# yycho0108/qpwcnet

Hardware: AMD Instinct MI355X
Metric: image-pairs/sec at 256x512 fp32 (higher is better)
Workload: dtype f32; 1 GPU; BASELINE configs[1]: full 6-level PWC-Net (qpwcnet build_flower) inference, batch 8 per GPU, 256x512 fp32, channels_last, d=4 cost volume + WarpV2; global_batch=8, batch_per_gpu=8, parallelism=dp1 (pairs sharded, RCCL all-gather of the 6 per-level EPE), hipgraph=True

## Files before the change

qpwcnet_amd/csrc/encoder.hip:

```cpp
#include "common.h"
#include "launch.h"

namespace qpwc {

__device__ __forceinline__ float enc_mishf(float x) {
    const float e = __builtin_amdgcn_exp2f(fminf(x, 20.0f) * 1.4426950408889634f);
    const float t = e * (e + 2.0f);
    const float m = x * (t * __builtin_amdgcn_rcpf(t + 2.0f));
    return m;
}

typedef float f32x4e __attribute__((ext_vector_type(4)));

__device__ __forceinline__ float2 ld2(const float* p) { return *reinterpret_cast<const float2*>(p); }
__device__ __forceinline__ float2 ld2(const __half* p) { return __half22float2(*reinterpret_cast<const __half2*>(p)); }
__device__ __forceinline__ void st4q(float* p, float4 v) { *reinterpret_cast<float4*>(p) = v; }
__device__ __forceinline__ void st4q(__half* p, float4 v) {
    __half2 lo = __floats2half2_rn(v.x, v.y), hi = __floats2half2_rn(v.z, v.w);
    uint2 u;
    u.x = *reinterpret_cast<unsigned*>(&lo);
    u.y = *reinterpret_cast<unsigned*>(&hi);
    *reinterpret_cast<uint2*>(p) = u;
}

constexpr int kEcTH = 8, kEcTW = 16;
constexpr int kEcHW = kEcTW + 2, kEcNH = (kEcTH + 2) * kEcHW;

template <int C>
__device__ __forceinline__ int ec_slot(int q, int hp) {
    return C == 16 ? (q ^ ((hp >> 2) & 3)) : (q ^ ((hp >> 1) & (C / 4 - 1)));
}

#ifndef QPWC_ENC_NT
#define QPWC_ENC_NT 1
#endif
#ifndef QPWC_UPCONV16_NFB_MIN_WGS
#define QPWC_UPCONV16_NFB_MIN_WGS 512
#endif
#ifndef QPWC_UPCONV256_TH
#define QPWC_UPCONV256_TH 2
#endif
#ifndef QPWC_UPCONV128_TH
#define QPWC_UPCONV128_TH 4
#endif
#ifndef QPWC_UPCONV64_LDS_TOTAL
#define QPWC_UPCONV64_LDS_TOTAL 82944
#endif
#ifndef QPWC_W_NEXT_ALWAYS
#define QPWC_W_NEXT_ALWAYS 1
#endif
#ifndef QPWC_W_NEXT_ALWAYS_F16
#define QPWC_W_NEXT_ALWAYS_F16 0
#endif
#if QPWC_W_NEXT_ALWAYS
#define QPWC_LOAD_W_NEXT(END) load_w(wn, kb + 1 < (END) ? kb + 1 : kb)
#else
#define QPWC_LOAD_W_NEXT(END) do { if (kb + 1 < (END)) load_w(wn, kb + 1); } while (0)
#endif
#ifdef QPWC_ENC_STAMP
__device__ long long g_enc_census[4096 * 6];
#define ENC_CENSUS(i) do { if (census_on) census_p[i] = __builtin_amdgcn_s_memtime(); } while (0)
#else
#define ENC_CENSUS(i) do { } while (0)
#endif
template <int C, int NT>
__global__ __launch_bounds__(256, 4) void conv3x3_mish_kernel(const float* __restrict__ x,
                                                              const float* __restrict__ weight,
                                                              const float* __restrict__ bias,
                                                              float* __restrict__ out, int H, int W,
                                                              int pad_h, int pad_w, int tiles_x, int tiles_y,
                                                              int groups_x) {
    constexpr int NQ = C / 4;
    constexpr int NFT = C / 16;
    constexpr int NKC = C / 16;
    constexpr int NLD = (kEcNH * NQ + 255) / 256;
    constexpr int NBUF = NT > 1 ? 2 : 1;
    __shared__ __attribute__((aligned(16))) float in_s[NBUF * kEcNH * C];
    const int tid0 = threadIdx.x;
    const int wave = __builtin_amdgcn_readfirstlane(tid0 >> 6);
    const int lane = tid0 & 63, n0 = lane & 15, g0 = lane >> 4;
    const int grp = xcd_swizzle(blockIdx.x, gridDim.x);
    const int gx0 = grp % groups_x, ty = (grp / groups_x) % tiles_y, b = grp / (groups_x * tiles_y);
    const int tx0 = gx0 * NT;
    const int Y0 = ty * kEcTH;
    const float* xb = x + (int64_t)b * H * W * C;
    const int Ho = H + pad_h, Wo = W + pad_w;
    float* ob = out + (int64_t)b * Ho * Wo * C;

    auto stage_load = [&](int tid, int tx, float4 (&v)[NLD]) {
        const int X0 = tx * kEcTW;
#pragma unroll
        for (int it = 0; it < NLD; ++it) {
            const int idx = tid + 256 * it;
            const int hp = idx / NQ, q = idx - hp * NQ;
            const int hy = hp / kEcHW, hx = hp - hy * kEcHW;
            const int gy = Y0 - 1 + hy, gx = X0 - 1 + hx;
            v[it] = (idx < kEcNH * NQ && gy >= 0 && gy < H && gx >= 0 && gx < W)
                        ? *reinterpret_cast<const float4*>(xb + ((int64_t)gy * W + gx) * C + 4 * q)
                        : make_float4(0.f, 0.f, 0.f, 0.f);
        }
    };
    auto stage_write = [&](int tid, int buf, const float4 (&v)[NLD]) {
#pragma unroll
        for (int it = 0; it < NLD; ++it) {
            const int idx = tid + 256 * it;
            const int hp = idx / NQ, q = idx - hp * NQ;
            if (idx < kEcNH * NQ)
                *reinterpret_cast<float4*>(in_s + buf * (kEcNH * C) + hp * C + 4 * ec_slot<C>(q, hp)) = v[it];
        }
    };
#ifdef QPWC_ENC_STAMP
    const bool census_on = tid0 == 0 && blockIdx.x < 4096;
    long long* census_p = g_enc_census + (blockIdx.x < 4096 ? blockIdx.x : 0) * 6;
    if (census_on)
        census_p[5] = (long long)(unsigned)__builtin_amdgcn_s_getreg((4) | (0 << 6) | (31 << 11)) |
                      ((long long)(unsigned)__builtin_amdgcn_s_getreg((20) | (0 << 6) | (31 << 11)) << 32);
#endif
    ENC_CENSUS(0);
    float4 st[NLD];
    stage_load(tid0, tx0, st);
#ifdef QPWC_ENC_STAMP
    asm volatile("s_waitcnt vmcnt(0)" ::: "memory");
#endif
    ENC_CENSUS(1);
    stage_write(tid0, 0, st);
    __syncthreads();
    ENC_CENSUS(2);

#pragma unroll 1
    for (int t = 0; t < NT; ++t) {
        const int tx = tx0 + t;
        if (tx >= tiles_x) break;
        const bool more = t + 1 < NT && tx + 1 < tiles_x;

        const int X0 = tx * kEcTW;
        const float* tile_s = in_s + (t & (NBUF - 1)) * (kEcNH * C);
        const float* wt = weight;
        int n = n0, g = g0, tid = tid0;
        if (NT > 1) asm volatile("" : "+r"(wt), "+v"(n), "+v"(g), "+v"(tid));
        if (more) stage_load(tid, tx + 1, st);
#pragma unroll
        for (int ft = 0; ft < NFT; ++ft) {
            f32x4e wld[9][NKC];
#pragma unroll
            for (int k = 0; k < 9; ++k)
#pragma unroll
                for (int kc = 0; kc < NKC; ++kc)
                    wld[k][kc] = *reinterpret_cast<const f32x4e*>(wt + ((int64_t)k * C + 16 * ft + n) * C + 16 * kc + 4 * g);
            f32x4e acc[2];
            acc[0] = f32x4e{0.f, 0.f, 0.f, 0.f};
            acc[1] = f32x4e{0.f, 0.f, 0.f, 0.f};
#pragma unroll
            for (int ky = 0; ky < 3; ++ky)
#pragma unroll
                for (int kx = 0; kx < 3; ++kx)
#pragma unroll
                    for (int kc = 0; kc < NKC; ++kc) {
                        f32x4e bv[2];
#pragma unroll
                        for (int m = 0; m < 2; ++m) {
                            const int hp = (2 * wave + m + ky) * kEcHW + n + kx;
                            const int q = 4 * kc + g;
                            const int slot = ec_slot<C>(q, hp);
                            bv[m] = *reinterpret_cast<const f32x4e*>(tile_s + hp * C + 4 * slot);
                        }
#pragma unroll
                        for (int tt = 0; tt < 4; ++tt)
#pragma unroll
                            for (int m = 0; m < 2; ++m)
                                acc[m] = __builtin_amdgcn_mfma_f32_16x16x4f32(wld[ky * 3 + kx][kc][tt], bv[m][tt], acc[m], 0, 0, 0);
                    }
            if (ft == NFT - 1) ENC_CENSUS(3);
            const float4 bq = *reinterpret_cast<const float4*>(bias + 16 * ft + 4 * g);
#pragma unroll
            for (int m = 0; m < 2; ++m) {
                const int gy = Y0 + 2 * wave + m, gx = X0 + n;
                if (gy < H && gx < W)
                    *reinterpret_cast<float4*>(ob + ((int64_t)gy * Wo + gx) * C + 16 * ft + 4 * g) =
                        make_float4(enc_mishf(acc[m][0] + bq.x), enc_mishf(acc[m][1] + bq.y),
                                    enc_mishf(acc[m][2] + bq.z), enc_mishf(acc[m][3] + bq.w));
            }
        }
        if (pad_w > 0 && X0 + kEcTW >= W) {
            for (int i = tid; i < kEcTH * pad_w * NQ; i += 256) {
                const int q = i % NQ, r = i / NQ, col = r % pad_w, row = r / pad_w;
                const int gy = Y0 + row;
                if (gy < H) *reinterpret_cast<float4*>(ob + ((int64_t)gy * Wo + W + col) * C + 4 * q) = make_float4(0.f, 0.f, 0.f, 0.f);
            }
        }
        if (pad_h > 0 && Y0 + kEcTH >= H) {
            const int x_end = (X0 + kEcTW >= W) ? Wo : X0 + kEcTW;
            for (int i = tid; i < pad_h * (x_end - X0) * NQ; i += 256) {
                const int q = i % NQ, r = i / NQ, col = r % (x_end - X0), row = r / (x_end - X0);
                *reinterpret_cast<float4*>(ob + ((int64_t)(H + row) * Wo + X0 + col) * C + 4 * q) = make_float4(0.f, 0.f, 0.f, 0.f);
            }
        }
        ENC_CENSUS(4);
        if (more) {
            stage_write(tid, (t + 1) & (NBUF - 1), st);
            __syncthreads();
        }
    }
}

constexpr int kEwSlots = 5;
constexpr unsigned kEwOob = 0x80000000u;

template <int C, int TH>
struct EwShape {
    static constexpr int NKB = C / 32;
    static constexpr int NS = 9 * NKB;
    static constexpr int NH = (TH + 2) * kEcHW;
    static constexpr int NHI = (NH * 8 + 255) / 256;
    static constexpr int HBLK = 4 * NHI * 1024;
    static constexpr int WBASE = 2 * HBLK;
    static constexpr int LDS = WBASE + 4 * kEwSlots * 2048;
    static_assert(NKB % 2 == 0, "the K-loop walks pairs of 32-channel blocks");
};

__device__ __forceinline__ void ew_wait_vm(int n) {
    switch (n) {
#define EW_W(k) case k: asm volatile("s_waitcnt vmcnt(" #k ")" ::: "memory"); break;
        EW_W(1) EW_W(2) EW_W(3) EW_W(4) EW_W(5) EW_W(6) EW_W(7) EW_W(8) EW_W(9) EW_W(10) EW_W(11) EW_W(12)
#undef EW_W
        default: asm volatile("s_waitcnt vmcnt(0)" ::: "memory"); break;
    }
}

__device__ __forceinline__ void ew_dma16(__amdgpu_buffer_rsrc_t r, char* lds, unsigned voff, int soff) {
#ifdef __HIP_DEVICE_COMPILE__
    typedef __attribute__((address_space(3))) void* lds_ptr_t;
    __builtin_amdgcn_raw_ptr_buffer_load_lds(r, (lds_ptr_t)lds, 16, voff, soff, 0, 0);
#endif
}

__device__ __forceinline__ void ew_pin_agpr(f32x4e& v) {
#ifdef __HIP_DEVICE_COMPILE__
    asm volatile("" : "+a"(v));
#endif
}

template <int C, int TH>
__global__ __launch_bounds__(256, (2 * EwShape<C, TH>::LDS <= 160 * 1024) ? 2 : 1) void conv3x3_mish_ring_kernel(
    const float* __restrict__ x, const float* __restrict__ weight, const float* __restrict__ bias,
    float* __restrict__ out, int H, int W, int pad_h, int pad_w, int tiles_x, int tiles_y, int n_tiles) {
    using S = EwShape<C, TH>;
    __shared__ __attribute__((aligned(1024))) char smem[S::LDS];
    const int tid = threadIdx.x;
    const int wave = __builtin_amdgcn_readfirstlane(tid >> 6);
    const int lane = tid & 63, n = lane & 15, g = lane >> 4;
    const int slice = blockIdx.x / n_tiles;
    const int tile = xcd_swizzle(blockIdx.x % n_tiles, n_tiles);
    const int tx = tile % tiles_x, ty = (tile / tiles_x) % tiles_y, b = tile / (tiles_x * tiles_y);
    const int X0 = tx * kEcTW, Y0 = ty * TH;
    const int fo = 64 * slice + 16 * wave;
    const __amdgpu_buffer_rsrc_t rx = __builtin_amdgcn_make_buffer_rsrc(
        const_cast<float*>(x) + (int64_t)b * H * W * C, 0, H * W * C * 4, 0x00020000);
    const __amdgpu_buffer_rsrc_t rw = __builtin_amdgcn_make_buffer_rsrc(const_cast<float*>(weight), 0, 9 * C * C * 4, 0x00020000);

    unsigned hoff[S::NHI];
#pragma unroll
    for (int j = 0; j < S::NHI; ++j) {
        const int i = (wave * S::NHI + j) * 64 + lane;
        const int hp = i >> 3, q = (i & 7) ^ (hp & 7);
        const int hy = hp / kEcHW, hx = hp - hy * kEcHW;
        const int gy = Y0 - 1 + hy, gx = X0 - 1 + hx;
        hoff[j] = (hp < S::NH && gy >= 0 && gy < H && gx >= 0 && gx < W) ? (unsigned)(((gy * W + gx) * C + 4 * q) * 4) : kEwOob;
    }
    const unsigned woff = (unsigned)(((fo + n) * C + 4 * g) * 4);
    auto issue_h = [&](int kb) __attribute__((always_inline)) {
#pragma unroll
        for (int j = 0; j < S::NHI; ++j)
            ew_dma16(rx, smem + (kb & 1) * S::HBLK + (wave * S::NHI + j) * 1024, hoff[j], kb * 128);
    };
    auto issue_w = [&](int s) __attribute__((always_inline)) {
        const int sc = s < S::NS ? s : S::NS - 1;
        const int kb = sc / 9, tap = sc - 9 * kb;
        char* dst = smem + S::WBASE + ((s % kEwSlots) * 4 + wave) * 2048;
#pragma unroll
        for (int kc = 0; kc < 2; ++kc)
            ew_dma16(rw, dst + kc * 1024, woff, (tap * C * C + 32 * kb + 16 * kc) * 4);
    };
    f32x4e wa[2][2], pb[2][2][TH];
    auto read = [&](int s, int buf) __attribute__((always_inline)) {
        const int kb = s / 9, tap = s - 9 * kb, ky = tap / 3, kx = tap - 3 * ky;
        const char* ws = smem + S::WBASE + ((s % kEwSlots) * 4 + wave) * 2048 + lane * 16;
        const char* hs = smem + (kb & 1) * S::HBLK;
#pragma unroll
        for (int kc = 0; kc < 2; ++kc) {
            wa[buf][kc] = *reinterpret_cast<const f32x4e*>(ws + kc * 1024);
#pragma unroll
            for (int m = 0; m < TH; ++m) {
                const int hp = (m + ky) * kEcHW + n + kx;
                pb[buf][kc][m] = *reinterpret_cast<const f32x4e*>(hs + hp * 128 + 16 * ((4 * kc + g) ^ (hp & 7)));
            }
        }
    };
    f32x4e acc[TH];
#pragma unroll
    for (int m = 0; m < TH; ++m) {
        acc[m] = f32x4e{0.f, 0.f, 0.f, 0.f};
        ew_pin_agpr(acc[m]);
    }

    issue_h(0);
#pragma unroll
    for (int s = 0; s < kEwSlots - 1; ++s) issue_w(s);
    ew_wait_vm(2 * (kEwSlots - 2));
    __builtin_amdgcn_s_barrier();
    read(0, 0);

    auto pair = [&](int p, const bool LAST) __attribute__((always_inline)) {
#pragma unroll
        for (int t = 0; t < 18; ++t) {
            const int s = 18 * p + t;
            const bool more = !(LAST && t == 17);
            if (more) {
                const int tb = t % 9;
                const bool h_young = tb >= 1 && tb <= kEwSlots - 2 && !(LAST && t >= 9);
                ew_wait_vm(2 * (kEwSlots - 3) + (h_young ? S::NHI : 0));
                if (tb == 8) {
                    asm volatile("s_waitcnt lgkmcnt(0)" ::: "memory");
                    __builtin_amdgcn_s_barrier();
                }
            }
            issue_w(s + kEwSlots - 1);
            if (t == 0) issue_h(2 * p + 1);
            if (t == 9 && !LAST) issue_h(2 * p + 2);
            if (more) read(s + 1, (t + 1) & 1);
            __builtin_amdgcn_sched_barrier(0);
#pragma unroll
            for (int kc = 0; kc < 2; ++kc)
#pragma unroll
                for (int tt = 0; tt < 4; ++tt)
#pragma unroll
                    for (int m = 0; m < TH; ++m)
                        acc[m] = __builtin_amdgcn_mfma_f32_16x16x4f32(wa[t & 1][kc][tt], pb[t & 1][kc][m][tt], acc[m], 0, 0, 0);
#pragma unroll
            for (int m = 0; m < TH; ++m) ew_pin_agpr(acc[m]);
            __builtin_amdgcn_sched_barrier(0);
        }
    };
#pragma unroll 1
    for (int p = 0; p < S::NKB / 2 - 1; ++p) pair(p, false);
    pair(S::NKB / 2 - 1, true);
    asm volatile("s_waitcnt vmcnt(0)" ::: "memory");

    const int Ho = H + pad_h, Wo = W + pad_w;
    float* ob = out + (int64_t)b * Ho * Wo * C;
    const float4 bq = *reinterpret_cast<const float4*>(bias + fo + 4 * g);
#pragma unroll
    for (int m = 0; m < TH; ++m) {
        const int gy = Y0 + m, gx = X0 + n;
        if (gy < H && gx < W)
            *reinterpret_cast<float4*>(ob + ((int64_t)gy * Wo + gx) * C + fo + 4 * g) =
                make_float4(enc_mishf(acc[m][0] + bq.x), enc_mishf(acc[m][1] + bq.y),
                            enc_mishf(acc[m][2] + bq.z), enc_mishf(acc[m][3] + bq.w));
    }
    if (pad_w > 0 && X0 + kEcTW >= W) {
        for (int i = tid; i < TH * pad_w * 16; i += 256) {
            const int q = i & 15, r = i >> 4, col = r % pad_w, row = r / pad_w;
            const int gy = Y0 + row;
            if (gy < H) *reinterpret_cast<float4*>(ob + ((int64_t)gy * Wo + W + col) * C + 64 * slice + 4 * q) = make_float4(0.f, 0.f, 0.f, 0.f);
        }
    }
    if (pad_h > 0 && Y0 + TH >= H) {
        const int x_end = (X0 + kEcTW >= W) ? Wo : X0 + kEcTW;
        for (int i = tid; i < pad_h * (x_end - X0) * 16; i += 256) {
            const int q = i & 15, r = i >> 4, col = r % (x_end - X0), row = r / (x_end - X0);
            *reinterpret_cast<float4*>(ob + ((int64_t)(H + row) * Wo + X0 + col) * C + 64 * slice + 4 * q) = make_float4(0.f, 0.f, 0.f, 0.f);
        }
    }
}

template <int C, int TH>
static int conv3x3_mish_ring_launch(const void* x, const void* weight, const void* bias, void* out, int B, int H,
                                    int W, int pad_h, int pad_w, hipStream_t s) {
    const int tiles_x = (W + kEcTW - 1) / kEcTW, tiles_y = (H + TH - 1) / TH;
    const int64_t n_tiles = (int64_t)tiles_x * tiles_y * B;
    if (n_tiles * (C / 64) > INT32_MAX || (int64_t)H * W * C * 4 > INT32_MAX) {
        set_error("conv3x3_mish: too many tiles or a frame of 2 GiB or more");
        return QPWC_E_SHAPE;
    }
    hipLaunchKernelGGL((conv3x3_mish_ring_kernel<C, TH>), dim3((unsigned)(n_tiles * (C / 64))), dim3(256), 0, s,
                       (const float*)x, (const float*)weight, (const float*)bias, (float*)out, H, W, pad_h, pad_w,
                       tiles_x, tiles_y, (int)n_tiles);
    return check_launch("conv3x3_mish_ring_kernel");
}

typedef _Float16 f16x8e __attribute__((ext_vector_type(8)));
typedef _Float16 f16x4e __attribute__((ext_vector_type(4)));

template <int CP>
__device__ __forceinline__ int f16_slot(int q, int hp) {
    return CP == 32 ? (q ^ ((0 - (hp >> 2)) & 3)) : (CP == 64 ? (q ^ ((hp >> 1) & 7)) : (q ^ (hp & 15)));
}

template <int C, int TH>
__global__ __launch_bounds__(256) void conv3x3_mish_f16_kernel(const __half* __restrict__ x,
                                                              const __half* __restrict__ weight,
                                                              const float* __restrict__ bias,
                                                              __half* __restrict__ out, int H, int W, int pad_h,
                                                              int pad_w, int tiles_x, int tiles_y, int n_tiles) {
    constexpr int CP = C < 32 ? 32 : C;
    constexpr int NQ = CP / 8, NQG = C / 8;
    constexpr int HH = TH + 2, NH = HH * kEcHW;
    constexpr int NKB = CP / 32;
    constexpr int FW = C < 64 ? C : 64, NFT = FW / 16, NSL = C / FW;
    constexpr int RW = TH / 4;
    constexpr int NST = (NH * NQ + 255) / 256;
    __shared__ __attribute__((aligned(16))) __half in_s[NH * CP];
    const int tid = threadIdx.x;
    const int wave = __builtin_amdgcn_readfirstlane(tid >> 6);
    const int lane = tid & 63, n = lane & 15, g = lane >> 4;
    const int slice = blockIdx.x / n_tiles;
    const int tile = xcd_swizzle(blockIdx.x % n_tiles, n_tiles);
    const int tx = tile % tiles_x, ty = (tile / tiles_x) % tiles_y, b = tile / (tiles_x * tiles_y);
    const int X0 = tx * kEcTW, Y0 = ty * TH;
    const int f0 = FW * slice;
    const __half* xb = x + (int64_t)b * H * W * C;
    {
        uint4 st[NST];
#pragma unroll
        for (int it = 0; it < NST; ++it) {
            const int idx = tid + 256 * it;
            const int hp = idx / NQ, q = idx - hp * NQ;
            const int hy = hp / kEcHW, hx = hp - hy * kEcHW;
            const int gy = Y0 - 1 + hy, gx = X0 - 1 + hx;
            st[it] = (idx < NH * NQ && q < NQG && gy >= 0 && gy < H && gx >= 0 && gx < W)
                         ? *reinterpret_cast<const uint4*>(xb + ((int64_t)gy * W + gx) * C + 8 * q)
                         : make_uint4(0u, 0u, 0u, 0u);
        }
#pragma unroll
        for (int it = 0; it < NST; ++it) {
            const int idx = tid + 256 * it;
            const int hp = idx / NQ, q = idx - hp * NQ;
            if (idx < NH * NQ) *reinterpret_cast<uint4*>(in_s + hp * CP + 8 * f16_slot<CP>(q, hp)) = st[it];
        }
    }
    const int Ho = H + pad_h, Wo = W + pad_w;
    __half* ob = out + (int64_t)b * Ho * Wo * C;
    if (C >= 64) {
        const int fo = f0 + 16 * wave;
        f32x4e acw[TH];
#pragma unroll
        for (int r = 0; r < TH; ++r) acw[r] = f32x4e{0.f, 0.f, 0.f, 0.f};
        f16x8e wv[9], wn[9];
        auto load_w = [&](f16x8e (&w)[9], int kb) {
#pragma unroll
            for (int tap = 0; tap < 9; ++tap)
                w[tap] = *reinterpret_cast<const f16x8e*>(weight + ((int64_t)tap * C + fo + n) * C + 32 * kb + 8 * g);
        };
        load_w(wv, 0);
        __syncthreads();
        auto block = [&](f16x8e (&wv)[9], int kb) __attribute__((always_inline)) {
            f16x8e bb[2][TH];
            auto read_b = [&](f16x8e (&bv)[TH], int tap) __attribute__((always_inline)) {
                const int ky = tap / 3, kx = tap - 3 * ky;
#pragma unroll
                for (int r = 0; r < TH; ++r) {
                    const int hp = (r + ky) * kEcHW + n + kx;
                    bv[r] = *reinterpret_cast<const f16x8e*>(in_s + hp * CP + 8 * f16_slot<CP>(4 * kb + g, hp));
                }
            };
            read_b(bb[0], 0);
#pragma unroll
            for (int tap = 0; tap < 9; ++tap) {
                if (tap + 1 < 9) read_b(bb[(tap + 1) & 1], tap + 1);
#pragma unroll
                for (int r = 0; r < TH; ++r)
                    acw[r] = __builtin_amdgcn_mfma_f32_16x16x32_f16(wv[tap], bb[tap & 1][r], acw[r], 0, 0, 0);
                __builtin_amdgcn_sched_barrier(0);
            }
        };
#if QPWC_W_NEXT_ALWAYS_F16
        {
            int kb = 0;
#pragma unroll 1
            for (; kb + 1 < NKB; kb += 2) {
                load_w(wn, kb + 1);
                __builtin_amdgcn_sched_barrier(0);
                block(wv, kb);
                load_w(wv, kb + 2 < NKB ? kb + 2 : kb);
                __builtin_amdgcn_sched_barrier(0);
                block(wn, kb + 1);
            }
            if (kb < NKB) block(wv, kb);
        }
#else
#pragma unroll 1
        for (int kb = 0; kb < NKB; ++kb) {
            if (kb + 1 < NKB) load_w(wn, kb + 1);
            block(wv, kb);
#pragma unroll
            for (int tap = 0; tap < 9; ++tap) wv[tap] = wn[tap];
        }
#endif
        const float4 bq = *reinterpret_cast<const float4*>(bias + fo + 4 * g);
#pragma unroll
        for (int r = 0; r < TH; ++r) {
            const int gy = Y0 + r, gx = X0 + n;
            if (gy < H && gx < W) {
                f16x4e o;
                o[0] = (_Float16)enc_mishf(acw[r][0] + bq.x);
                o[1] = (_Float16)enc_mishf(acw[r][1] + bq.y);
                o[2] = (_Float16)enc_mishf(acw[r][2] + bq.z);
                o[3] = (_Float16)enc_mishf(acw[r][3] + bq.w);
                *reinterpret_cast<f16x4e*>(ob + ((int64_t)gy * Wo + gx) * C + fo + 4 * g) = o;
            }
        }
    } else {
    f32x4e acc[RW][NFT];
#pragma unroll
    for (int r = 0; r < RW; ++r)
#pragma unroll
        for (int ft = 0; ft < NFT; ++ft) acc[r][ft] = f32x4e{0.f, 0.f, 0.f, 0.f};
    __syncthreads();
    const bool kvalid = 8 * g < C;
#pragma unroll 1
    for (int kb = 0; kb < NKB; ++kb) {
#pragma unroll
        for (int tap = 0; tap < 9; ++tap) {
            const int ky = tap / 3, kx = tap - 3 * ky;
            f16x8e wv[NFT];
#pragma unroll
            for (int ft = 0; ft < NFT; ++ft) {
                wv[ft] = f16x8e{0, 0, 0, 0, 0, 0, 0, 0};
                if (kvalid)
                    wv[ft] = *reinterpret_cast<const f16x8e*>(weight + ((int64_t)tap * C + f0 + 16 * ft + n) * C + 32 * kb + 8 * g);
            }
            f16x8e bv[RW];
#pragma unroll
            for (int r = 0; r < RW; ++r) {
                const int hp = (RW * wave + r + ky) * kEcHW + n + kx;
                bv[r] = *reinterpret_cast<const f16x8e*>(in_s + hp * CP + 8 * f16_slot<CP>(4 * kb + g, hp));
            }
#pragma unroll
            for (int ft = 0; ft < NFT; ++ft)
#pragma unroll
                for (int r = 0; r < RW; ++r)
                    acc[r][ft] = __builtin_amdgcn_mfma_f32_16x16x32_f16(wv[ft], bv[r], acc[r][ft], 0, 0, 0);
        }
    }
    float4 bqs[NFT];
#pragma unroll
    for (int ft = 0; ft < NFT; ++ft) bqs[ft] = *reinterpret_cast<const float4*>(bias + f0 + 16 * ft + 4 * g);
#pragma unroll
    for (int ft = 0; ft < NFT; ++ft) {
        const float4 bq = bqs[ft];
#pragma unroll
        for (int r = 0; r < RW; ++r) {
            const int gy = Y0 + RW * wave + r, gx = X0 + n;
            if (gy < H && gx < W) {
                f16x4e o;
                o[0] = (_Float16)enc_mishf(acc[r][ft][0] + bq.x);
                o[1] = (_Float16)enc_mishf(acc[r][ft][1] + bq.y);
                o[2] = (_Float16)enc_mishf(acc[r][ft][2] + bq.z);
                o[3] = (_Float16)enc_mishf(acc[r][ft][3] + bq.w);
                *reinterpret_cast<f16x4e*>(ob + ((int64_t)gy * Wo + gx) * C + f0 + 16 * ft + 4 * g) = o;
            }
        }
    }
    }
    constexpr int NQF = FW / 8;
    if (pad_w > 0 && X0 + kEcTW >= W) {
        for (int i = tid; i < TH * pad_w * NQF; i += 256) {
            const int q = i % NQF, r = i / NQF, col = r % pad_w, row = r / pad_w;
            const int gy = Y0 + row;
            if (gy < H) *reinterpret_cast<uint4*>(ob + ((int64_t)gy * Wo + W + col) * C + f0 + 8 * q) = make_uint4(0u, 0u, 0u, 0u);
        }
    }
    if (pad_h > 0 && Y0 + TH >= H) {
        const int x_end = (X0 + kEcTW >= W) ? Wo : X0 + kEcTW;
        for (int i = tid; i < pad_h * (x_end - X0) * NQF; i += 256) {
            const int q = i % NQF, r = i / NQF, col = r % (x_end - X0), row = r / (x_end - X0);
            *reinterpret_cast<uint4*>(ob + ((int64_t)(H + row) * Wo + X0 + col) * C + f0 + 8 * q) = make_uint4(0u, 0u, 0u, 0u);
        }
    }
    (void)NSL;
}

template <int C>
__device__ __forceinline__ int f16n_slot(int q, int hp) {
    return C == 16 ? (q ^ ((hp >> 3) & 1)) : (q ^ ((0 - (hp >> 2)) & 3));
}

template <int C>
__global__ __launch_bounds__(256, C == 16 ? 4 : 3) void conv3x3_mish_f16_narrow_kernel(
    const __half* __restrict__ x, const __half* __restrict__ weight, const float* __restrict__ bias,
    __half* __restrict__ out, int H, int W, int pad_h, int pad_w, int tiles_x, int tiles_y) {
    constexpr int TH = 16, RW = 4, HWD = kEcTW + 2;
    constexpr int NQ = C / 8, NH = (TH + 2) * HWD;
    constexpr int NST = (NH * NQ + 255) / 256;
    constexpr int NFT = C / 16;
    __shared__ __attribute__((aligned(16))) __half in_s[NH * C];
    const int tid = threadIdx.x;
    const int wave = __builtin_amdgcn_readfirstlane(tid >> 6);
    const int lane = tid & 63, n = lane & 15, g = lane >> 4;
    const int tile = xcd_swizzle(blockIdx.x, gridDim.x);
    const int tx = tile % tiles_x, ty = (tile / tiles_x) % tiles_y, b = tile / (tiles_x * tiles_y);
    const int X0 = tx * kEcTW, Y0 = ty * TH;
    const __half* xb = x + (int64_t)b * H * W * C;
    const int Ho = H + pad_h, Wo = W + pad_w;
    __half* ob = out + (int64_t)b * Ho * Wo * C;
    {
        uint4 st[NST];
#pragma unroll
        for (int it = 0; it < NST; ++it) {
            const int idx = tid + 256 * it;
            const int hp = idx / NQ, q = idx - hp * NQ;
            const int hy = hp / HWD, hx = hp - hy * HWD;
            const int gy = Y0 - 1 + hy, gx = X0 - 1 + hx;
            st[it] = (idx < NH * NQ && gy >= 0 && gy < H && gx >= 0 && gx < W)
                         ? *reinterpret_cast<const uint4*>(xb + ((int64_t)gy * W + gx) * C + 8 * q)
                         : make_uint4(0u, 0u, 0u, 0u);
        }
#pragma unroll
        for (int it = 0; it < NST; ++it) {
            const int idx = tid + 256 * it;
            const int hp = idx / NQ, q = idx - hp * NQ;
            if (idx < NH * NQ) *reinterpret_cast<uint4*>(in_s + hp * C + 8 * f16n_slot<C>(q, hp)) = st[it];
        }
    }
    constexpr int NS = C == 16 ? 5 : 9;
    const int gh = C == 16 ? (g >> 1) : 0, gq = C == 16 ? (g & 1) : g;
    f16x8e wv[NS][NFT];
#pragma unroll
    for (int j = 0; j < NS; ++j) {
        const int tap = C == 16 ? 2 * j + gh : j;
#pragma unroll
        for (int ft = 0; ft < NFT; ++ft) {
            wv[j][ft] = f16x8e{0, 0, 0, 0, 0, 0, 0, 0};
            if (tap < 9) wv[j][ft] = *reinterpret_cast<const f16x8e*>(weight + ((int64_t)tap * C + 16 * ft + n) * C + 8 * gq);
        }
    }
    f32x4e acc[RW][NFT];
#pragma unroll
    for (int r = 0; r < RW; ++r)
#pragma unroll
        for (int ft = 0; ft < NFT; ++ft) acc[r][ft] = f32x4e{0.f, 0.f, 0.f, 0.f};
    __syncthreads();
    f16x8e bb[2][RW];
    auto read_b = [&](f16x8e (&bv)[RW], int j) __attribute__((always_inline)) {
        const int t0 = C == 16 ? 2 * j + gh : j;
        const int tap = t0 < 9 ? t0 : 8;
        const int ky = tap / 3, kx = tap - 3 * ky;
#pragma unroll
        for (int r = 0; r < RW; ++r) {
            const int hp = (RW * wave + r + ky) * HWD + n + kx;
            bv[r] = *reinterpret_cast<const f16x8e*>(in_s + hp * C + 8 * f16n_slot<C>(gq, hp));
        }
    };
    read_b(bb[0], 0);
#pragma unroll
    for (int j = 0; j < NS; ++j) {
        if (j + 1 < NS) read_b(bb[(j + 1) & 1], j + 1);
#pragma unroll
        for (int ft = 0; ft < NFT; ++ft)
#pragma unroll
            for (int r = 0; r < RW; ++r)
                acc[r][ft] = __builtin_amdgcn_mfma_f32_16x16x32_f16(wv[j][ft], bb[j & 1][r], acc[r][ft], 0, 0, 0);
        __builtin_amdgcn_sched_barrier(0);
    }
    float4 bqs[NFT];
#pragma unroll
    for (int ft = 0; ft < NFT; ++ft) bqs[ft] = *reinterpret_cast<const float4*>(bias + 16 * ft + 4 * g);
#pragma unroll
    for (int ft = 0; ft < NFT; ++ft) {
        const float4 bq = bqs[ft];
#pragma unroll
        for (int r = 0; r < RW; ++r) {
            const int gy = Y0 + RW * wave + r, gx = X0 + n;
            if (gy < H && gx < W) {
                f16x4e o;
                o[0] = (_Float16)enc_mishf(acc[r][ft][0] + bq.x);
                o[1] = (_Float16)enc_mishf(acc[r][ft][1] + bq.y);
                o[2] = (_Float16)enc_mishf(acc[r][ft][2] + bq.z);
                o[3] = (_Float16)enc_mishf(acc[r][ft][3] + bq.w);
                *reinterpret_cast<f16x4e*>(ob + ((int64_t)gy * Wo + gx) * C + 16 * ft + 4 * g) = o;
            }
        }
    }
    if (pad_w > 0 && X0 + kEcTW >= W) {
        for (int i = tid; i < TH * pad_w * NQ; i += 256) {
            const int q = i % NQ, r = i / NQ, col = r % pad_w, row = r / pad_w;
            const int gy = Y0 + row;
            if (gy < H) *reinterpret_cast<uint4*>(ob + ((int64_t)gy * Wo + W + col) * C + 8 * q) = make_uint4(0u, 0u, 0u, 0u);
        }
    }
    if (pad_h > 0 && Y0 + TH >= H) {
// ... 543 lines not shown
            if (gy < Ho && gx < Wo)
                *reinterpret_cast<float4*>(ob + ((int64_t)gy * Wo + gx) * CO + 16 * ft + 4 * g) =
                    make_float4(enc_mishf(acc[m][ft][0] + bq.x), enc_mishf(acc[m][ft][1] + bq.y),
                                enc_mishf(acc[m][ft][2] + bq.z), enc_mishf(acc[m][ft][3] + bq.w));
        }
    }
}

template <int CI, int TH>
__global__ __launch_bounds__(256, (2 * (2 * TH + 1) * (kEcTW + 1) * CI * 4 > 80 * 1024) ? 1 : 2) void conv3x3s2_mish_wide_kernel(const float* __restrict__ x,
                                                                     const float* __restrict__ weight,
                                                                     const float* __restrict__ bias,
                                                                     float* __restrict__ out, int H, int W,
                                                                     int tiles_x, int tiles_y, int n_tiles) {
    constexpr int CO = 2 * CI, NQ = CI / 4, NKB = CI / 32;
    constexpr int IH = 2 * TH + 1, PW = kEcTW + 1;
    constexpr int NPX = IH * 33;
    constexpr int NST = (NPX * NQ + 255) / 256;
    __shared__ __attribute__((aligned(16))) float in_s[2 * IH * PW * CI];
    const int tid = threadIdx.x;
    const int wave = __builtin_amdgcn_readfirstlane(tid >> 6);
    const int lane = tid & 63, n = lane & 15, g = lane >> 4;
    const int slice = blockIdx.x / n_tiles;
    const int tile = xcd_swizzle(blockIdx.x % n_tiles, n_tiles);
    const int tx = tile % tiles_x, ty = (tile / tiles_x) % tiles_y, b = tile / (tiles_x * tiles_y);
    const int X0 = tx * kEcTW, Y0 = ty * TH;
    const int Hp = H + 1, Wp = W + 1, Ho = H / 2, Wo = W / 2;
    const int fo = 64 * slice + 16 * wave;
    const float* xb = x + (int64_t)b * Hp * Wp * CI;
    auto slot = [](int q, int pix) { return CI == 32 ? (q ^ ((pix >> 1) & 7)) : (q ^ (pix & 15)); };
    constexpr int kChunk = NST;
#pragma unroll
    for (int base = 0; base < NST; base += kChunk) {
        float4 st[kChunk];
#pragma unroll
        for (int i = 0; i < kChunk; ++i) {
            const int idx = tid + 256 * (base + i);
            const int pxl = idx / NQ, q = idx - pxl * NQ;
            const int row = pxl / 33, col = pxl - row * 33;
            const int gy = 2 * Y0 + row, gx = 2 * X0 + col;
            st[i] = (base + i < NST && idx < NPX * NQ && gy < Hp && gx < Wp)
                        ? *reinterpret_cast<const float4*>(xb + ((int64_t)gy * Wp + gx) * CI + 4 * q)
                        : make_float4(0.f, 0.f, 0.f, 0.f);
        }
#pragma unroll
        for (int i = 0; i < kChunk; ++i) {
            const int idx = tid + 256 * (base + i);
            const int pxl = idx / NQ, q = idx - pxl * NQ;
            const int row = pxl / 33, col = pxl - row * 33;
            const int pix = ((col & 1) * IH + row) * PW + (col >> 1);
            if (base + i < NST && idx < NPX * NQ) *reinterpret_cast<float4*>(in_s + pix * CI + 4 * slot(q, pix)) = st[i];
        }
    }
    f32x4e acc[TH];
#pragma unroll
    for (int m = 0; m < TH; ++m) acc[m] = f32x4e{0.f, 0.f, 0.f, 0.f};
    f32x4e wv[9][2], wn[9][2];
    auto load_w = [&](f32x4e (&w)[9][2], int kb) {
#pragma unroll
        for (int k = 0; k < 9; ++k)
#pragma unroll
            for (int kc = 0; kc < 2; ++kc)
                w[k][kc] = *reinterpret_cast<const f32x4e*>(weight + ((int64_t)k * CO + fo + n) * CI + 32 * kb + 16 * kc + 4 * g);
    };
    load_w(wv, 0);
    __syncthreads();
    auto block = [&](f32x4e (&wv)[9][2], int kb) __attribute__((always_inline)) {
#pragma unroll
        for (int ky = 0; ky < 3; ++ky)
#pragma unroll
            for (int kx = 0; kx < 3; ++kx)
#pragma unroll
                for (int kc = 0; kc < 2; ++kc) {
                    f32x4e bv[TH];
#pragma unroll
                    for (int m = 0; m < TH; ++m) {
                        const int pix = ((kx & 1) * IH + 2 * m + ky) * PW + n + (kx >> 1);
                        bv[m] = *reinterpret_cast<const f32x4e*>(in_s + pix * CI + 4 * slot(8 * kb + 4 * kc + g, pix));
                    }
#pragma unroll
                    for (int t = 0; t < 4; ++t)
#pragma unroll
                        for (int m = 0; m < TH; ++m)
                            acc[m] = __builtin_amdgcn_mfma_f32_16x16x4f32(wv[ky * 3 + kx][kc][t], bv[m][t], acc[m], 0, 0, 0);
                }
    };
#if QPWC_W_NEXT_ALWAYS
    {
        int kb = 0;
#pragma unroll 1
        for (; kb + 1 < NKB; kb += 2) {
            load_w(wn, kb + 1);
            __builtin_amdgcn_sched_barrier(0);
            block(wv, kb);
            load_w(wv, kb + 2 < NKB ? kb + 2 : kb);
            __builtin_amdgcn_sched_barrier(0);
            block(wn, kb + 1);
        }
        if (kb < NKB) block(wv, kb);
    }
#else
#pragma unroll 1
    for (int kb = 0; kb < NKB; ++kb) {
        if (kb + 1 < NKB) load_w(wn, kb + 1);
        block(wv, kb);
#pragma unroll
        for (int k = 0; k < 9; ++k)
#pragma unroll
            for (int kc = 0; kc < 2; ++kc) wv[k][kc] = wn[k][kc];
    }
#endif
    float* ob = out + (int64_t)b * Ho * Wo * CO;
    const float4 bq = *reinterpret_cast<const float4*>(bias + fo + 4 * g);
#pragma unroll
    for (int m = 0; m < TH; ++m) {
        const int gy = Y0 + m, gx = X0 + n;
        if (gy < Ho && gx < Wo)
            *reinterpret_cast<float4*>(ob + ((int64_t)gy * Wo + gx) * CO + fo + 4 * g) =
                make_float4(enc_mishf(acc[m][0] + bq.x), enc_mishf(acc[m][1] + bq.y),
                            enc_mishf(acc[m][2] + bq.z), enc_mishf(acc[m][3] + bq.w));
    }
}

template <int CI, int TH>
static int conv3x3s2_mish_wide_launch(const void* x, const void* weight, const void* bias, void* out, int B,
                                      int H, int W, hipStream_t s) {
    const int tiles_x = (W / 2 + kEcTW - 1) / kEcTW, tiles_y = (H / 2 + TH - 1) / TH;
    const int64_t n_tiles = (int64_t)tiles_x * tiles_y * B;
    const int slices = 2 * CI / 64;
    if (n_tiles * slices > INT32_MAX) {
        set_error("conv3x3s2_mish: too many tiles");
        return QPWC_E_SHAPE;
    }
    hipLaunchKernelGGL((conv3x3s2_mish_wide_kernel<CI, TH>), dim3((unsigned)(n_tiles * slices)), dim3(256), 0, s,
                       (const float*)x, (const float*)weight, (const float*)bias, (float*)out, H, W, tiles_x, tiles_y,
                       (int)n_tiles);
    return check_launch("conv3x3s2_mish_wide_kernel");
}

int conv3x3s2_mish_any_launch(const void* x, const void* weight, const void* bias, void* out, int B, int H, int W,
                              int CI, hipStream_t s);

int conv3x3s2_mish_launch(const void* x, const void* weight, const void* bias, void* out, int B, int H, int W,
                          hipStream_t s) {
    const int tiles_x = (W / 2 + kEcTW - 1) / kEcTW, tiles_y = (H / 2 + kEcTH - 1) / kEcTH;
    const int64_t nblk = (int64_t)tiles_x * tiles_y * B;
    if (nblk > INT32_MAX) {
        set_error("conv3x3s2_mish: too many tiles");
        return QPWC_E_SHAPE;
    }
    hipLaunchKernelGGL(conv3x3s2_mish_kernel, dim3((unsigned)nblk), dim3(256), 0, s, (const float*)x,
                       (const float*)weight, (const float*)bias, (float*)out, H, W, tiles_x, tiles_y);
    return check_launch("conv3x3s2_mish_kernel");
}

int conv3x3s2_mish_any_launch(const void* x, const void* weight, const void* bias, void* out, int B, int H, int W,
                              int CI, hipStream_t s) {
    switch (CI) {
        case 16: return conv3x3s2_mish_launch(x, weight, bias, out, B, H, W, s);
        case 32: return conv3x3s2_mish_wide_launch<32, 4>(x, weight, bias, out, B, H, W, s);
        case 64: return conv3x3s2_mish_wide_launch<64, 2>(x, weight, bias, out, B, H, W, s);
        case 128: return conv3x3s2_mish_wide_launch<128, 2>(x, weight, bias, out, B, H, W, s);
        default: set_error("conv3x3s2_mish: C_in=%d not in {16,32,64,128}", CI); return QPWC_E_SHAPE;
    }
}

template <int CI, int TH>
__global__ __launch_bounds__(256) void conv3x3s2_mish_f16_kernel(const __half* __restrict__ x,
                                                                const __half* __restrict__ weight,
                                                                const float* __restrict__ bias,
                                                                __half* __restrict__ out, int H, int W, int tiles_x,
                                                                int tiles_y, int n_tiles) {
    constexpr int CO = 2 * CI;
    constexpr int CP = CI < 32 ? 32 : CI;
    constexpr int NQ = CP / 8, NQG = CI / 8, NKB = CP / 32;
    constexpr int IH = 2 * TH + 1, PW = kEcTW + 1;
    constexpr int NB = CO / 16;
    constexpr int WB = NB < 4 ? NB : 4, WR = 4 / WB;
    constexpr int RW = TH / WR;
    constexpr int NCH = IH * (2 * kEcTW + 1) * NQ;
    constexpr int NST = (NCH + 255) / 256;
    __shared__ __attribute__((aligned(16))) __half in_s[2 * IH * PW * CP];
    const int tid = threadIdx.x;
    const int wave = __builtin_amdgcn_readfirstlane(tid >> 6);
    const int lane = tid & 63, n = lane & 15, g = lane >> 4;
    const int slice = blockIdx.x / n_tiles;
    const int tile = xcd_swizzle(blockIdx.x % n_tiles, n_tiles);
    const int tx = tile % tiles_x, ty = (tile / tiles_x) % tiles_y, b = tile / (tiles_x * tiles_y);
    const int X0 = tx * kEcTW, Y0 = ty * TH;
    const int Hp = H + 1, Wp = W + 1, Ho = H / 2, Wo = W / 2;
    const __half* xb = x + (int64_t)b * Hp * Wp * CI;
    {
        uint4 st[NST];
#pragma unroll
        for (int it = 0; it < NST; ++it) {
            const int idx = tid + 256 * it;
            const int q = idx % NQ, pc = idx / NQ;
            const int row = pc / (2 * kEcTW + 1), col = pc - row * (2 * kEcTW + 1);
            const int gy = 2 * Y0 + row, gx = 2 * X0 + col;
            st[it] = (idx < NCH && q < NQG && gy < Hp && gx < Wp)
                         ? *reinterpret_cast<const uint4*>(xb + ((int64_t)gy * Wp + gx) * CI + 8 * q)
                         : make_uint4(0u, 0u, 0u, 0u);
        }
#pragma unroll
        for (int it = 0; it < NST; ++it) {
            const int idx = tid + 256 * it;
            const int q = idx % NQ, pc = idx / NQ;
            const int row = pc / (2 * kEcTW + 1), col = pc - row * (2 * kEcTW + 1);
            const int hp = ((col & 1) * IH + row) * PW + (col >> 1);
            if (idx < NCH) *reinterpret_cast<uint4*>(in_s + hp * CP + 8 * f16_slot<CP>(q, hp)) = st[it];
        }
    }
    const int blk = WB == 4 ? 4 * slice + wave : (wave % WB);
    const int r0 = WB == 4 ? 0 : (wave / WB) * RW;
    const int fo = 16 * blk;
    f32x4e acc[RW];
#pragma unroll
    for (int r = 0; r < RW; ++r) acc[r] = f32x4e{0.f, 0.f, 0.f, 0.f};
    const bool kvalid = 8 * g < CI;
    f16x8e wv[9], wn[9];
    auto load_w = [&](f16x8e (&w)[9], int kb) {
#pragma unroll
        for (int tap = 0; tap < 9; ++tap) {
            w[tap] = f16x8e{0, 0, 0, 0, 0, 0, 0, 0};
            if (kvalid) w[tap] = *reinterpret_cast<const f16x8e*>(weight + ((int64_t)tap * CO + fo + n) * CI + 32 * kb + 8 * g);
        }
    };
    load_w(wv, 0);
    __syncthreads();
    auto block = [&](f16x8e (&wv)[9], int kb) __attribute__((always_inline)) {
#pragma unroll
        for (int tap = 0; tap < 9; ++tap) {
            const int ky = tap / 3, kx = tap - 3 * ky;
#pragma unroll
            for (int r = 0; r < RW; ++r) {
                const int hp = ((kx & 1) * IH + 2 * (r0 + r) + ky) * PW + n + (kx >> 1);
                const f16x8e bv = *reinterpret_cast<const f16x8e*>(in_s + hp * CP + 8 * f16_slot<CP>(4 * kb + g, hp));
                acc[r] = __builtin_amdgcn_mfma_f32_16x16x32_f16(wv[tap], bv, acc[r], 0, 0, 0);
            }
        }
    };
#if QPWC_W_NEXT_ALWAYS_F16
    {
        int kb = 0;
#pragma unroll 1
        for (; kb + 1 < NKB; kb += 2) {
            load_w(wn, kb + 1);
            __builtin_amdgcn_sched_barrier(0);
            block(wv, kb);
            load_w(wv, kb + 2 < NKB ? kb + 2 : kb);
            __builtin_amdgcn_sched_barrier(0);
            block(wn, kb + 1);
        }
        if (kb < NKB) block(wv, kb);
    }
#else
#pragma unroll 1
    for (int kb = 0; kb < NKB; ++kb) {
        if (kb + 1 < NKB) load_w(wn, kb + 1);
        block(wv, kb);
#pragma unroll
        for (int tap = 0; tap < 9; ++tap) wv[tap] = wn[tap];
    }
#endif
    __half* ob = out + (int64_t)b * Ho * Wo * CO;
    const float4 bq = *reinterpret_cast<const float4*>(bias + fo + 4 * g);
#pragma unroll
    for (int r = 0; r < RW; ++r) {
        const int gy = Y0 + r0 + r, gx = X0 + n;
        if (gy < Ho && gx < Wo)
            st4q(ob + ((int64_t)gy * Wo + gx) * CO + fo + 4 * g,
                 make_float4(enc_mishf(acc[r][0] + bq.x), enc_mishf(acc[r][1] + bq.y), enc_mishf(acc[r][2] + bq.z),
                             enc_mishf(acc[r][3] + bq.w)));
    }
}

template <int CI, int TH>
static int conv3x3s2_mish_f16_launch_t(const void* x, const void* weight, const void* bias, void* out, int B, int H,
                                       int W, hipStream_t s) {
    constexpr int NSL = (2 * CI / 16) < 4 ? 1 : (2 * CI / 16) / 4;
    const int tiles_x = (W / 2 + kEcTW - 1) / kEcTW, tiles_y = (H / 2 + TH - 1) / TH;
    const int64_t n_tiles = (int64_t)tiles_x * tiles_y * B;
    if (n_tiles * NSL > INT32_MAX) {
        set_error("conv3x3s2_mish_f16: too many tiles");
        return QPWC_E_SHAPE;
    }
    hipLaunchKernelGGL((conv3x3s2_mish_f16_kernel<CI, TH>), dim3((unsigned)(n_tiles * NSL)), dim3(256), 0, s,
                       (const __half*)x, (const __half*)weight, (const float*)bias, (__half*)out, H, W, tiles_x,
                       tiles_y, (int)n_tiles);
    return check_launch("conv3x3s2_mish_f16_kernel");
}

int conv3x3s2_mish_f16_launch(const void* x, const void* weight, const void* bias, void* out, int B, int H, int W,
                              int CI, hipStream_t s) {
    switch (CI) {
        case 16: return conv3x3s2_mish_f16_launch_t<16, 8>(x, weight, bias, out, B, H, W, s);
        case 32: return conv3x3s2_mish_f16_launch_t<32, 8>(x, weight, bias, out, B, H, W, s);
        case 64: return conv3x3s2_mish_f16_launch_t<64, 4>(x, weight, bias, out, B, H, W, s);
        case 128: return conv3x3s2_mish_f16_launch_t<128, 2>(x, weight, bias, out, B, H, W, s);
        default: set_error("conv3x3s2_mish_f16: C_in=%d not in {16,32,64,128}", CI); return QPWC_E_SHAPE;
    }
}

int conv3x3_mish_launch(const void* x, const void* weight, const void* bias, void* out, int B, int H, int W,
                        int C, int pad_h, int pad_w, hipStream_t s) {
    const int tiles_x = (W + kEcTW - 1) / kEcTW, tiles_y = (H + kEcTH - 1) / kEcTH;
    constexpr int NT = QPWC_ENC_NT;
    const int groups_x = (tiles_x + NT - 1) / NT;
    const int64_t nblk = (int64_t)groups_x * tiles_y * B;
    if (nblk > INT32_MAX) {
        set_error("conv3x3_mish: too many tiles");
        return QPWC_E_SHAPE;
    }
    const dim3 grid((unsigned)nblk);
    if (C == 16)
        hipLaunchKernelGGL((conv3x3_mish_kernel<16, NT>), grid, dim3(256), 0, s, (const float*)x, (const float*)weight,
                           (const float*)bias, (float*)out, H, W, pad_h, pad_w, tiles_x, tiles_y, groups_x);
    else if (C == 32)
        hipLaunchKernelGGL((conv3x3_mish_kernel<32, NT>), grid, dim3(256), 0, s, (const float*)x, (const float*)weight,
                           (const float*)bias, (float*)out, H, W, pad_h, pad_w, tiles_x, tiles_y, groups_x);
    else if (C == 64)
        return conv3x3_mish_ring_launch<64, 4>(x, weight, bias, out, B, H, W, pad_h, pad_w, s);
    else if (C == 128)
        return conv3x3_mish_ring_launch<128, 4>(x, weight, bias, out, B, H, W, pad_h, pad_w, s);
    else if (C == 256)
        return conv3x3_mish_ring_launch<256, 2>(x, weight, bias, out, B, H, W, pad_h, pad_w, s);
    else {
        set_error("conv3x3_mish: C=%d not in {16,32,64,128,256}", C);
        return QPWC_E_SHAPE;
    }
    return check_launch("conv3x3_mish_kernel");
}

}

#ifdef QPWC_ENC_STAMP
extern "C" int qpwc_debug_enc_census(long long* out, int n) {
    if (n > 4096 * 6) n = 4096 * 6;
    return (int)hipMemcpyFromSymbol(out, HIP_SYMBOL(qpwc::g_enc_census), n * sizeof(long long), 0, hipMemcpyDeviceToHost);
}
#endif
```

Baseline: 7327 pairs/s.

## Add persistent double-buffered MFMA conv3x3 Mish kernel for 16/32 channels

Adds a persistent-grid kernel for the C=16 and C=32 fp32 3x3 conv+Mish layers. Each workgroup loops over tiles and prefetches the next tile's halo into a second LDS slot via buffer DMA while computing the current one. Weights stay in registers and f32 MFMA 16x16x4 runs with swizzled LDS reads. The grid is capped at CUs times a fixed per-CU workgroup count. The aim is to hide global-load latency and cut launch and weight-reload overhead on the high-resolution encoder layers, at the cost of higher register pressure and an occupancy tied to the hard-coded per-CU workgroup count.

```diff
diff --git a/qpwcnet_amd/csrc/encoder.hip b/qpwcnet_amd/csrc/encoder.hip
--- a/qpwcnet_amd/csrc/encoder.hip
+++ b/qpwcnet_amd/csrc/encoder.hip
@@ -1,3 +1,5 @@
+#include <atomic>
+
 #include "common.h"
 #include "launch.h"
 
@@ -386,6 +388,182 @@
                        (const float*)x, (const float*)weight, (const float*)bias, (float*)out, H, W, pad_h, pad_w,
                        tiles_x, tiles_y, (int)n_tiles);
     return check_launch("conv3x3_mish_ring_kernel");
+}
+
+constexpr int kEnWgPerCu16 = 4;
+constexpr int kEnWgPerCu32 = 3;
+
+template <int C>
+struct EnShape {
+    static constexpr int WGS = C == 16 ? kEnWgPerCu16 : kEnWgPerCu32;
+    static constexpr int TH = C == 16 ? 8 : 4;
+    static constexpr int NQ = C / 4, NFT = C / 16, NKC = C / 16;
+    static constexpr int NH = (TH + 2) * kEcHW;
+    static constexpr int NP = (NH * NQ + 255) / 256;
+    static constexpr int SLOT = 4 * NP * 1024;
+    static constexpr int NST = 2;
+    static_assert(TH * NFT == 8, "four waves x two tile rows x one output block");
+};
+
+template <int C>
+__device__ __forceinline__ int en_slot(int q, int hp) {
+    return C == 16 ? (q ^ ((hp >> 1) & 2)) : (q ^ (hp & 7));
+}
+
+__device__ __forceinline__ void en_store16(__amdgpu_buffer_rsrc_t r, unsigned voff, float4 v) {
+#ifdef __HIP_DEVICE_COMPILE__
+    typedef unsigned en_u32x4 __attribute__((ext_vector_type(4)));
+    en_u32x4 u;
+    u[0] = __float_as_uint(v.x), u[1] = __float_as_uint(v.y), u[2] = __float_as_uint(v.z), u[3] = __float_as_uint(v.w);
+    __builtin_amdgcn_raw_buffer_store_b128(u, r, voff, 0, 0);
+#endif
+}
+
+template <int C>
+__global__ __launch_bounds__(256, EnShape<C>::WGS) void conv3x3_mish_nring_kernel(
+    const float* __restrict__ x, const float* __restrict__ weight, const float* __restrict__ bias,
+    float* __restrict__ out, int H, int W, int pad_h, int pad_w, int tiles_x, int tiles_y, int n_tiles) {
+    using S = EnShape<C>;
+    __shared__ __attribute__((aligned(1024))) char smem[2 * S::SLOT];
+    const int tid = threadIdx.x;
+    const int wave = __builtin_amdgcn_readfirstlane(tid >> 6);
+    const int lane = tid & 63, n_ = lane & 15, g_ = lane >> 4;
+    const int ft = wave % S::NFT, r0 = 2 * (wave / S::NFT);
+    const int Ho = H + pad_h, Wo = W + pad_w;
+
+    struct Tile {
+        int X0, Y0, b;
+        bool live;
+    };
+    auto locate = [&](int i) __attribute__((always_inline)) {
+        Tile t;
+        t.live = i < n_tiles;
+        const int tile = xcd_swizzle(t.live ? i : 0, n_tiles);
+        t.X0 = (tile % tiles_x) * kEcTW;
+        t.Y0 = ((tile / tiles_x) % tiles_y) * S::TH;
+        t.b = tile / (tiles_x * tiles_y);
+        return t;
+    };
+    int hpk[S::NP];
+#pragma unroll
+    for (int j = 0; j < S::NP; ++j) {
+        const int i = (wave * S::NP + j) * 64 + lane;
+        const int hp = i / S::NQ, q = en_slot<C>(i % S::NQ, hp);
+        const int hy = hp / kEcHW, hx = hp - hy * kEcHW;
+        hpk[j] = hp < S::NH ? (hy | hx << 8 | q << 16) : -1;
+    }
+    auto request = [&](const Tile& t, int slot) __attribute__((always_inline)) {
+        const __amdgpu_buffer_rsrc_t rx = __builtin_amdgcn_make_buffer_rsrc(
+            const_cast<float*>(x) + (int64_t)t.b * H * W * C, 0, t.live ? H * W * C * 4 : 0, 0x00020000);
+#pragma unroll
+        for (int j = 0; j < S::NP; ++j) {
+            const int gy = t.Y0 - 1 + (hpk[j] & 255), gx = t.X0 - 1 + ((hpk[j] >> 8) & 255), q = (hpk[j] >> 16) & 255;
+            unsigned off = (unsigned)(((gy * W + gx) * C + 4 * q) * 4);
+            asm volatile("" : "+v"(off));
+            const bool in = hpk[j] >= 0 && (unsigned)gy < (unsigned)H && (unsigned)gx < (unsigned)W;
+            ew_dma16(rx, smem + slot * S::SLOT + (wave * S::NP + j) * 1024, in ? off : kEwOob, 0);
+        }
+    };
+
+    f32x4e wld[9][S::NKC];
+#pragma unroll
+    for (int k = 0; k < 9; ++k)
+#pragma unroll
+        for (int kc = 0; kc < S::NKC; ++kc)
+            wld[k][kc] = *reinterpret_cast<const f32x4e*>(weight + ((int64_t)k * C + 16 * ft + n_) * C + 16 * kc + 4 * g_);
+    float4 bq = *reinterpret_cast<const float4*>(bias + 16 * ft + 4 * g_);
+
+    int ra[4][3];
+#pragma unroll
+    for (int rr = 0; rr < 4; ++rr)
+#pragma unroll
+        for (int kx = 0; kx < 3; ++kx) {
+            const int hp = (r0 + rr) * kEcHW + n_ + kx;
+            ra[rr][kx] = hp * (C * 4) + 16 * en_slot<C>(g_, hp);
+            asm volatile("" : "+v"(ra[rr][kx]));
+        }
+
+    auto compute = [&](const Tile& t, int slot) __attribute__((always_inline)) {
+        const int n = n_, g = g_;
+        f32x4e bv[2][2];
+        auto read = [&](int s, int buf) __attribute__((always_inline)) {
+            const int tap = s / S::NKC, kc = s - tap * S::NKC, ky = tap / 3, kx = tap - 3 * ky;
+#pragma unroll
+            for (int m = 0; m < 2; ++m)
+                bv[buf][m] = *reinterpret_cast<const f32x4e*>(smem + ((slot * S::SLOT + ra[m + ky][kx]) ^ (64 * kc)));
+        };
+        f32x4e acc[2];
+#pragma unroll
+        for (int m = 0; m < 2; ++m) {
+            acc[m] = f32x4e{0.f, 0.f, 0.f, 0.f};
+            ew_pin_agpr(acc[m]);
+        }
+        read(0, 0);
+#pragma unroll
+        for (int s = 0; s < 9 * S::NKC; ++s) {
+            if (s + 1 < 9 * S::NKC) read(s + 1, (s + 1) & 1);
+            __builtin_amdgcn_sched_barrier(0);
+#pragma unroll
+            for (int tt = 0; tt < 4; ++tt)
+#pragma unroll
+                for (int m = 0; m < 2; ++m)
+                    acc[m] = __builtin_amdgcn_mfma_f32_16x16x4f32(wld[s / S::NKC][s % S::NKC][tt], bv[s & 1][m][tt], acc[m], 0, 0, 0);
+            ew_pin_agpr(acc[0]);
+            ew_pin_agpr(acc[1]);
+            __builtin_amdgcn_sched_barrier(0);
+        }
+        float* ob = out + (int64_t)t.b * Ho * Wo * C;
+        if (pad_w > 0 && t.X0 + kEcTW >= W) {
+            for (int i = tid; i < S::TH * pad_w * S::NQ; i += 256) {
+                const int q = i % S::NQ, r = i / S::NQ, col = r % pad_w, row = r / pad_w;
+                const int gy = t.Y0 + row;
+                if (gy < H) *reinterpret_cast<float4*>(ob + ((int64_t)gy * Wo + W + col) * C + 4 * q) = make_float4(0.f, 0.f, 0.f, 0.f);
+            }
+        }
+        if (pad_h > 0 && t.Y0 + S::TH >= H) {
+            const int x_end = (t.X0 + kEcTW >= W) ? Wo : t.X0 + kEcTW;
+            for (int i = tid; i < pad_h * (x_end - t.X0) * S::NQ; i += 256) {
+                const int q = i % S::NQ, r = i / S::NQ, col = r % (x_end - t.X0), row = r / (x_end - t.X0);
+                *reinterpret_cast<float4*>(ob + ((int64_t)(H + row) * Wo + t.X0 + col) * C + 4 * q) = make_float4(0.f, 0.f, 0.f, 0.f);
+            }
+        }
+        const __amdgpu_buffer_rsrc_t ro = __builtin_amdgcn_make_buffer_rsrc(ob, 0, Ho * Wo * C * 4, 0x00020000);
+        __builtin_amdgcn_sched_barrier(0);
+#pragma unroll
+        for (int m = 0; m < 2; ++m) {
+            const int gy = t.Y0 + r0 + m, gx = t.X0 + n;
+            en_store16(ro, (gy < H && gx < W) ? (unsigned)(((gy * Wo + gx) * C + 16 * ft + 4 * g) * 4) : kEwOob,
+                       make_float4(enc_mishf(acc[m][0] + bq.x), enc_mishf(acc[m][1] + bq.y),
+                                   enc_mishf(acc[m][2] + bq.z), enc_mishf(acc[m][3] + bq.w)));
+        }
+        __builtin_amdgcn_sched_barrier(0);
+    };
+
+    int i = blockIdx.x;
+    Tile cur = locate(i), nxt = locate(i + (int)gridDim.x);
+    request(cur, 0);
+    request(nxt, 1);
+#pragma unroll
+    for (int k = 0; k < 9; ++k)
+#pragma unroll
+        for (int kc = 0; kc < S::NKC; ++kc) asm volatile("" : "+v"(wld[k][kc]));
+    asm volatile("" : "+v"(bq.x), "+v"(bq.y), "+v"(bq.z), "+v"(bq.w));
+    ew_wait_vm(S::NP);
+    asm volatile("s_waitcnt lgkmcnt(0)" ::: "memory");
+    __builtin_amdgcn_s_barrier();
+    compute(cur, 0);
+#pragma unroll 1
+    for (int k = 1; nxt.live; ++k) {
+        cur = nxt;
+        i += (int)gridDim.x;
+        nxt = locate(i + (int)gridDim.x);
+        ew_wait_vm(S::NST);
+        asm volatile("s_waitcnt lgkmcnt(0)" ::: "memory");
+        __builtin_amdgcn_s_barrier();
+        request(nxt, (k + 1) & 1);
+        compute(cur, k & 1);
+    }
+    asm volatile("s_waitcnt vmcnt(0)" ::: "memory");
 }
 
 typedef _Float16 f16x8e __attribute__((ext_vector_type(8)));
@@ -1535,8 +1713,43 @@
     }
 }
 
+static int device_cus() {
+    static std::atomic<int> known[64];
+    int dev = 0, cus = 0;
+    if (hipGetDevice(&dev) != hipSuccess || dev < 0 || dev >= 64) return 0;
+    if ((cus = known[dev].load(std::memory_order_relaxed)) > 0) return cus;
+    if (hipDeviceGetAttribute(&cus, hipDeviceAttributeMultiprocessorCount, dev) != hipSuccess || cus < 0) return 0;
+    known[dev].store(cus, std::memory_order_relaxed);
+    return cus;
+}
+
+template <int C>
+static bool conv3x3_mish_nring_fits(int B, int H, int W, int pad_h, int pad_w) {
+    const int64_t tiles = (int64_t)((W + kEcTW - 1) / kEcTW) * ((H + EnShape<C>::TH - 1) / EnShape<C>::TH) * B;
+    return (int64_t)(H + pad_h) * (W + pad_w) * C * 4 <= INT32_MAX && tiles <= INT32_MAX / 2;
+}
+
+template <int C>
+static void conv3x3_mish_nring_launch(const void* x, const void* weight, const void* bias, void* out, int B, int H,
+                                      int W, int pad_h, int pad_w, hipStream_t s) {
+    const int tiles_x = (W + kEcTW - 1) / kEcTW, tiles_y = (H + EnShape<C>::TH - 1) / EnShape<C>::TH;
+    const int n_tiles = tiles_x * tiles_y * B;
+    const int cap = device_cus() * EnShape<C>::WGS;
+    hipLaunchKernelGGL((conv3x3_mish_nring_kernel<C>), dim3((unsigned)(cap > 0 && cap < n_tiles ? cap : n_tiles)),
+                       dim3(256), 0, s, (const float*)x, (const float*)weight, (const float*)bias, (float*)out, H, W,
+                       pad_h, pad_w, tiles_x, tiles_y, n_tiles);
+}
+
 int conv3x3_mish_launch(const void* x, const void* weight, const void* bias, void* out, int B, int H, int W,
                         int C, int pad_h, int pad_w, hipStream_t s) {
+    if (C == 16 && conv3x3_mish_nring_fits<16>(B, H, W, pad_h, pad_w)) {
+        conv3x3_mish_nring_launch<16>(x, weight, bias, out, B, H, W, pad_h, pad_w, s);
+        return check_launch("conv3x3_mish_kernel");
+    }
+    if (C == 32 && conv3x3_mish_nring_fits<32>(B, H, W, pad_h, pad_w)) {
+        conv3x3_mish_nring_launch<32>(x, weight, bias, out, B, H, W, pad_h, pad_w, s);
+        return check_launch("conv3x3_mish_kernel");
+    }
     const int tiles_x = (W + kEcTW - 1) / kEcTW, tiles_y = (H + kEcTH - 1) / kEcTH;
     constexpr int NT = QPWC_ENC_NT;
     const int groups_x = (tiles_x + NT - 1) / NT;
```

Measured after the change: 7371 pairs/s, median of 6. Within noise of the previous version (+0.6%).
